# wangchou/whisper.coreml

Hardware: AMD Instinct MI355X
Metric: xRT (audio-s/s) large-v3 beam=5 @1/2/4/8 GPU; p50 per-token decode ms (higher is better)
Workload: dtype fp16; 1 GPU; large-v3 beam=5 transcribe() of one 600 s file, 30 s clip grid, condition_on_previous_text=False, temperature=0; model=large-v3, global_batch=20, seq_len=448

## Files before the change

### include/whisper_hip.h

```cpp
#ifndef WHISPER_HIP_H
#define WHISPER_HIP_H
#include <stdint.h>

#ifdef __cplusplus
extern "C" {
#endif

typedef struct wh_ctx wh_ctx;

typedef struct wh_dims {
  int n_mels, n_audio_ctx, n_audio_state, n_audio_head, n_audio_layer;
  int n_vocab, n_text_ctx, n_text_state, n_text_head, n_text_layer;
} wh_dims;

enum { WH_F32 = 0, WH_F16 = 1 };

typedef struct wh_decode_opts {
  int group;
  int beam;
  float patience;
  float temperature;
  int sample_len;
  int suppress_blank;
  int timestamps;
// ... 46 lines not shown
int wh_mel_max_batch(wh_ctx* ctx, float* gmax, int n_files);
int wh_mel_read(wh_ctx* ctx, float* out, int64_t frame0, int64_t n_frames);
int wh_mel_write(wh_ctx* ctx, const float* mel, int64_t n_frames);

int wh_encode(wh_ctx* ctx, int n_win, const int64_t* seek_frames, const int* seg_frames);
int wh_read_audio_features(wh_ctx* ctx, int slot, float* out);
int wh_read_cross_kv(wh_ctx* ctx, int slot, int layer, float* k_out, float* v_out);

int wh_decode_begin(wh_ctx* ctx, int n_win, const wh_decode_opts* opts, const int* init_tokens, const int* n_init,
                    int max_init, const int* sot_index);
int wh_decode_begin_slots(wh_ctx* ctx, int n_win, const int* slots, const wh_decode_opts* opts,
                          const int* init_tokens, const int* n_init, int max_init, const int* sot_index);
int wh_decode_steps(wh_ctx* ctx, int max_steps, int* n_done);
int wh_decode_read(wh_ctx* ctx, int slot, int* tokens, float* sum_logprobs, int* len, int* fin_n, int* fin_tokens,
                   int* fin_len, float* fin_score, float* no_speech_prob);
int wh_decode_maxc(wh_ctx* ctx);

int wh_prefill(wh_ctx* ctx, int n_win, int group, const int* tokens, const int* n_tokens, int max_tokens,
               const int* sot_index, float* logits);
int wh_step(wh_ctx* ctx, const int* tokens, const int* text_offsets, float* logits);
int wh_reorder_kv(wh_ctx* ctx, const int* source_rows);

int wh_prefill_logits(wh_ctx* ctx, int slot, const int* tokens, int n_tokens, float* logits, const int* align_heads,
                      int n_align, float* align_qk);

int wh_align(wh_ctx* ctx, int slot, const int* tokens, int n_tokens, int n_sot, int num_frames, const int* align_heads,
             int n_align, int medfilt_width, float* token_probs, int* path, int* path_len);
int wh_align_batch(wh_ctx* ctx, int n_win, const int* slots, const int* tokens, const int* n_tokens, int n_sot,
                   const int* num_frames, const int* align_heads, int n_align, int medfilt_width, float* token_probs,
                   int* paths, int* path_lens);
// ... 43 lines not shown
```

### whisper.coreml_amd/csrc/wh_kernels.h

```cpp
#pragma once
#include "wh_common.h"

namespace wh {

constexpr int TKP = 1536;

template <typename T>
void launch_layernorm(const float* x, T* y, const float* g, const float* b, int rows, int n, float eps,
                      const int* rows_in, hipStream_t st);
template <typename T>
void launch_resid_ln(float* x, const float* part, int nsplit, int64_t part_stride, const float* bias, T* y,
                     const float* g, const float* b, int rows, int n, float eps, hipStream_t st, int slab_half = 0);
template <typename T>
void launch_attn_enc(const T* qkv, int ld, int ns, int H, int Tlen, int nwin, int64_t wsi, const T* vt, int tkp, T* out,
                     int64_t wso, hipStream_t st);
template <typename T>
void launch_self_attn(const T* q, int ldq, const T* kc, const T* vc, const int* rw, const int* rs, const int* rp,
                      const int* anc, int anc_beams, int nbeam, int H, int ctx, T* out, int ldo, int rows,
                      hipStream_t st);
template <typename T>
int launch_self_attn_qkv(const float* part, int nsplit, int64_t part_stride, const float* bqkv, int ns, T* kc, T* vc,
                          const int* rw, const int* rs, const int* rp, const int* anc, int anc_beams, int nbeam, int H,
                          int ctx, T* out, int ldo, int rows, hipStream_t st, int slab_half = 0);
template <typename T>
// ... 7 lines not shown
  const float* bias = nullptr;
  int max_rows = 0;
  float* split_rec = nullptr;
  int* split_cnt = nullptr;
  int max_pairs = 0;
  const void* qx = nullptr;
  const void* qwf = nullptr;
};
inline bool xattn_fused_q(int n, int rows_per_window, int elem_size) {
  return elem_size == 2 && n == 1280 && rows_per_window >= 1 && rows_per_window <= 8;
}
void launch_wq_frag(const void* w, void* f, int n, hipStream_t st);
constexpr int XREC = 16 * 64 + 32;
constexpr int XS_NSP = 24;
constexpr int XS_QP = 4;
int xattn_seg_grid(int npair, int nsp, int smax);
inline bool cross_attn_q_slabs(int z) { return z == 4 || z == 8 || z == 10; }
template <typename T>
void launch_cross_attn(const T* q, int ldq, const T* ck, const T* cv, int Tk, int H, int nsplit, int nwin,
                       const int* win_row0, const int* win_nrows, const int* win_slot, int64_t win_stride, float* po,
                       float* pm, float* pl, T* out, int ldo, int rows, float* qk_out, const int* qk_map, int qk_rows,
                       hipStream_t st, XQPart xq = XQPart());
template <typename T>
void launch_embed(const T* E, const T* P, int n, const int* row_tok, int* row_pos, const int* hist,
                  const int* cur_len, int G, int hctx, int pmax, float* x, int rows, hipStream_t st);
template <typename T>
void launch_mel_windows(const float* mel, int64_t ld_mel, int n_mels, const int64_t* seeks, const int* segs, T* melT,
                        int64_t win_stride, int rows_alloc, int nwin, hipStream_t st);
template <typename T>
void launch_zero_rows(T* buf, int64_t ws, int n, int ra, int rb, int nwin, hipStream_t st);

// ... 68 lines not shown
```

### whisper.coreml_amd/csrc/wh_kernels.hip

```cpp
#include "wh_kernels.h"

#include <cstdio>
#include <type_traits>
#include <cstdlib>

namespace wh {

template <typename T>
__global__ __launch_bounds__(256) void k_layernorm(const float* __restrict__ x, T* __restrict__ y, const float* __restrict__ gamma,
                                                   const float* __restrict__ beta, int rows, int n, float eps,
                                                   const int* __restrict__ rows_in) {
  const int row = blockIdx.x * 4 + (threadIdx.x >> 6);
  const int lane = threadIdx.x & 63;
  if (row >= rows) return;
  const int src = rows_in ? rows_in[row] : row;
  const float* xr = x + (int64_t)src * n;
  constexpr int MAXV = 8;
  float4_t v[MAXV];
  const int nv = n >> 2;
#pragma unroll
  for (int i = 0; i < MAXV; ++i) {
    const int c = lane + 64 * i;
    if (c < nv) v[i] = load4f(xr + 4 * c);
  }
// ... 538 lines not shown
    store4(op, o[0] * inv, o[1] * inv, o[2] * inv, o[3] * inv);
    store4(op + 4, o[4] * inv, o[5] * inv, o[6] * inv, o[7] * inv);
  }
  CT_END(CT_SELF_ATTN);
}

template <typename T>
void launch_self_attn(const T* q, int ldq, const T* kc, const T* vc, const int* rw, const int* rs, const int* rp,
                      const int* anc, int anc_beams, int nbeam, int H, int ctx, T* out, int ldo, int rows,
                      hipStream_t st) {
  if (rows <= 0) return;
  k_self_attn<T><<<dim3(rows, H), 64, 0, st>>>(q, ldq, kc, vc, rw, rs, rp, anc, anc_beams, nbeam, H, ctx, out, ldo,
                                               self_attn_kco_min()), wh_launched("k_self_attn");
}

template <typename T, typename S = float>
__global__ __launch_bounds__(64) __attribute__((amdgpu_waves_per_eu(1, 2))) void k_self_attn_qkv(const S* __restrict__ part, int nsplit, int64_t part_stride,
                                                      const float* __restrict__ bqkv, int ns, T* __restrict__ kc,
                                                      T* __restrict__ vc, const int* __restrict__ row_win,
                                                      const int* __restrict__ row_slot, const int* __restrict__ row_pos,
                                                      const int* __restrict__ anc, int anc_beams, int nbeam, int H,
                                                      int ctx, T* __restrict__ out, int ldo, int kco_min = 0) {
  __shared__ float sc[512];
  __shared__ int slot_of[512];
  __shared__ float qs[64], vs[64];
  const int lane = threadIdx.x, G = anc_beams;
  CT_MARK(CT_SELF_ATTN, 0);
  const int L = xcd_remap(blockIdx.x, gridDim.x), sl = L % G, wh = L / G, h = wh % H, w = wh / H, row = w * G + sl;
  const int* an = anc + ((int64_t)w * anc_beams + sl) * ctx;
  const int64_t head_stride = (int64_t)ctx * 64;
  const int64_t wbase = (int64_t)w * nbeam;
  auto kv_off = [&](int slot, int p) -> int64_t { return ((wbase + slot) * H + h) * head_stride + (int64_t)p * 64; };
  constexpr int TB = (int)sizeof(T), ROWB = 64 * TB;
  const int slotB = H * ctx * ROWB, baseB = ((int)wbase * H + h) * ctx * ROWB;
  const auto rk = wt_rsrc(kc), rv = wt_rsrc(vc);
  const int pos = row_pos[row];
  int sv[8];
#pragma unroll
  for (int i = 0; i < 8; ++i) sv[i] = an[min(lane + 64 * i, ctx - 1)];
  float qd, kd, vd;
  {
    constexpr bool H16 = sizeof(S) == 2;
    const S* pr = part + (int64_t)row * 3 * ns + h * 64 + lane;
    qd = bqkv[h * 64 + lane];
    kd = bqkv[ns + h * 64 + lane];
    vd = bqkv[2 * ns + h * 64 + lane];
    S a0[16], a1[16], a2[16];
#pragma unroll
    for (int z = 0; z < 16; ++z)
      if (H16 || z < nsplit) {
        const int64_t zo = (int64_t)(H16 ? min(z, nsplit - 1) : z) * part_stride;
        a0[z] = pr[zo];
        a1[z] = pr[zo + ns];
        a2[z] = pr[zo + 2 * ns];
      }
    if constexpr (H16) {
      asm volatile("" ::"s"(pos));
#pragma unroll
      for (int z = 0; z < 16; ++z) asm volatile("" ::"v"(a0[z]), "v"(a1[z]), "v"(a2[z]));
    }
    auto f32 = [](S r) -> float { return (float)r; };
#pragma unroll
    for (int z = 0; z < 16; ++z)
      if (z < nsplit) {
        qd += f32(a0[z]);
        kd += f32(a1[z]);
        vd += f32(a2[z]);
      }
  }
  for (int i = 0; i < 8; ++i)
    if (lane + 64 * i < pos) slot_of[lane + 64 * i] = sv[i] * slotB;
  const int plast = max(pos - 1, 0);
  const T qT = from_f32<T>(qd), kT = from_f32<T>(kd), vT = from_f32<T>(vd);
  kc[kv_off(sl, pos) + lane] = kT;
  vc[kv_off(sl, pos) + lane] = vT;
  qs[lane] = to_f32(qT);
  vs[lane] = to_f32(vT);
  const float s_cur = wave_sum(to_f32(qT) * to_f32(kT));
// ... 170 lines not shown
int self_attn_kco_min() {
  static const int v = [] {
    const char* e = tune_env("WHISPER_HIP_SA_KCO_MIN");
    return e ? atoi(e) : 64;
  }();
  return v;
}
template <typename T>
int launch_self_attn_qkv(const float* part, int nsplit, int64_t part_stride, const float* bqkv, int ns, T* kc, T* vc,
                          const int* rw, const int* rs, const int* rp, const int* anc, int anc_beams, int nbeam, int H,
                          int ctx, T* out, int ldo, int rows, hipStream_t st, int slab_half) {
  if (rows <= 0) return 0;
  if (anc_beams < 1 || rows % anc_beams || nsplit > 16) return -1;
  if (slab_half) {
    if constexpr (sizeof(T) == 2) {
      k_self_attn_qkv<T, half_t><<<rows * H, 64, 0, st>>>(reinterpret_cast<const half_t*>(part), nsplit, part_stride,
                                                         bqkv, ns, kc, vc, rw, rs, rp, anc, anc_beams, nbeam, H, ctx,
                                                         out, ldo, self_attn_kco_min()), wh_launched("k_self_attn_qkv");
      return 0;
    }
    return -1;
  }
  k_self_attn_qkv<T><<<rows * H, 64, 0, st>>>(part, nsplit, part_stride, bqkv, ns, kc, vc, rw, rs, rp, anc, anc_beams,
                                             nbeam, H, ctx, out, ldo, self_attn_kco_min()), wh_launched("k_self_attn_qkv");
  return 0;
}

template <typename T, int ACT, typename S = float>
__global__ __launch_bounds__(256) void k_reduce_store(const S* __restrict__ part, int nsplit, int64_t part_stride,
                                                      const float* __restrict__ bias, T* __restrict__ out, int ldo, int M,
                                                      int N) {
  const int i = (int)(blockIdx.x * 256 + threadIdx.x) * 4;
  CT_MARK(CT_REDUCE, 0);
// ... 340 lines not shown
  }
  XS_MARK(8);
  wh_lds_barrier();
  if (kh == 0) {
    const float* bl = reinterpret_cast<const float*>(xst + BIAS_OFF);
#pragma unroll
    for (int j = 0; j < XS_QF; ++j)
      if (j < np) {
        float4_t v = red2[(j * 4 + c) * 64 + lane] + red2[((XS_QF + j) * 4 + c) * 64 + lane];
        v += *reinterpret_cast<const float4_t*>(bl + j * 64 + c * 16 + 4 * g);
        store4(&qs[j][r][c * 16 + 4 * g], v[0], v[1], v[2], v[3]);
      }
  }
}

template <typename T, int QZ, int RR, typename S = float, bool FULL = false, int QK = 0>
__global__ __launch_bounds__(512, 1) void k_xattn_seg(const T* __restrict__ q, int ldq, const T* ck, const T* cvt, int Tk,
                                                     int H, int npair, int nsp, const int* __restrict__ win_row0,
                                                     const int* __restrict__ win_nrows,
                                                     const int* __restrict__ win_slot, int64_t win_stride, XQPart xq,
                                                     T* __restrict__ out, int ldo) {
  constexpr int NW = 8, SMAX = XsShape<RR>::SMAX, PPASS = 512 / (RR * 16);
  constexpr bool QP = QZ > 0;
  constexpr bool QF = QK > 0;
  __shared__ float seg_m[SMAX][RR], seg_l[SMAX][RR];
  __shared__ __attribute__((aligned(16))) float seg_o[SMAX][RR][68];
  __shared__ __attribute__((aligned(16))) T qs[XS_QP][16][72];
  __shared__ int s_ticket[2];
  __shared__ int s_wnr[XS_QP], s_wr0[XS_QP];
  const int tid = threadIdx.x, lane = tid & 63, wave = tid >> 6;
  const int r = lane & 15, g = lane >> 4;
// ... 186 lines not shown
  XS_MARK(3);

  typedef unsigned u32x4 __attribute__((ext_vector_type(4)));
  const auto rs = __builtin_amdgcn_make_buffer_rsrc(xq.split_rec, 0, 0x7fffffff, 0x00020000);
  const int part = tid / (RR * 16), t = tid - part * (RR * 16), qq = t >> 4, dc = (t & 15) * 4;
  auto emit = [&](int pj, const float4_t& o) {
    int wj, hj;
    pair_wh(pj, wj, hj);
    store4(out + (int64_t)(s_wr0[pj - pa] + qq) * ldo + hj * 64 + dc, o[0], o[1], o[2], o[3]);
  };
#pragma unroll
  for (int pass = 0; pass < (XS_QP + PPASS - 1) / PPASS; ++pass) {
    const int pj = pa + pass * PPASS + part;
    if (pj <= plast && qq < s_wnr[pj - pa]) {
      const int l0 = pj * nsp - s0, l1 = l0 + nsp;
      if (l0 >= 0 && l1 <= cnt) {
        emit(pj, xs_merge(nsp, [&](int k, float& m, float& l, float4_t& o) {
               m = seg_m[l0 + k][qq];
               l = seg_l[l0 + k][qq];
               o = *reinterpret_cast<const float4_t*>(&seg_o[l0 + k][qq][dc]);
             }));
      } else {
        for (int s = max(l0, 0); s < min(l1, cnt); ++s) {
          const int rb = (pj * nsp + (s - l0)) * XREC * 4;
          const float4_t o = *reinterpret_cast<const float4_t*>(&seg_o[s][qq][dc]);
          __builtin_amdgcn_raw_buffer_store_b128(__builtin_bit_cast(u32x4, o), rs, rb + (qq * 64 + dc) * 4, 0, 16);
          if (dc == 0) {
            __builtin_amdgcn_raw_buffer_store_b32(__builtin_bit_cast(unsigned, seg_m[s][qq]), rs, rb + (1024 + qq) * 4, 0, 16);
            __builtin_amdgcn_raw_buffer_store_b32(__builtin_bit_cast(unsigned, seg_l[s][qq]), rs, rb + (1040 + qq) * 4, 0, 16);
          }
        }
      }
    }
  }
  asm volatile("s_waitcnt vmcnt(0)" ::: "memory");
  __syncthreads();
  XS_MARK(4);
  const bool cut_a = pa * nsp < s0 || pa * nsp + nsp > s1;
  const bool cut_b = plast != pa && plast * nsp + nsp > s1;
  if (tid == 0) {
    const int ca = min(s1, pa * nsp + nsp) - s0, cb = s1 - plast * nsp;
    s_ticket[0] = cut_a && __hip_atomic_fetch_add(xq.split_cnt + pa, ca, __ATOMIC_RELAXED, __HIP_MEMORY_SCOPE_AGENT) + ca == nsp;
    s_ticket[1] = cut_b && __hip_atomic_fetch_add(xq.split_cnt + plast, cb, __ATOMIC_RELAXED, __HIP_MEMORY_SCOPE_AGENT) + cb == nsp;
  }
  __syncthreads();
  XS_MARK(5);
  CT_MARK(CT_XATTN, 3);
  if (part > 1 || !s_ticket[part]) return;
  __builtin_amdgcn_fence(__ATOMIC_ACQUIRE, "wavefront");
// ... 6 lines not shown
         l = __builtin_bit_cast(float, __builtin_amdgcn_raw_buffer_load_b32(rs, rb + (1040 + qq) * 4, 0, 16));
         o = __builtin_bit_cast(float4_t, __builtin_amdgcn_raw_buffer_load_b128(rs, rb + (qq * 64 + dc) * 4, 0, 16));
       }));
  XS_MARK(6);
}

#if WH_TUNING
}
WH_CT_READER(kernels)
extern "C" int wh_tune_xs_trace(unsigned long long* out) {
  return hipMemcpyFromSymbol(out, HIP_SYMBOL(wh::g_xs_trace), sizeof(wh::g_xs_trace)) == hipSuccess ? 0 : -1;
}
namespace wh {
#endif

int xattn_seg_grid(int npair, int nsp, int smax) {
  const int nseg = npair * nsp;
  int k = (nseg + 256 * 8 - 1) / (256 * 8), forced = 0;
  if (const char* e = tune_env("WHISPER_HIP_XS_K")) {
    const int v = atoi(e);
    if (v >= 1) k = v, forced = 1;
    if (v < 0) {
      const int nwg = std::min(-v, nseg);
      return (nseg + nwg - 1) / nwg > smax ? (nseg + smax - 1) / smax : nwg;
    }
  }
  if (!forced && npair >= 192) {
    const int ppw = (npair + 255) / 256, nwg = (npair + ppw - 1) / ppw;
    if (nwg >= 192 && ppw * nsp <= smax) return nwg;
  }
  if (k > smax / 8) k = smax / 8;
  int nwg = k == 1 ? (nseg < 200 ? nseg : 200) : (nseg + 8 * k - 1) / (8 * k);
  if ((nseg + nwg - 1) / nwg > smax) nwg = (nseg + smax - 1) / smax;
  return nwg;
}

__global__ __launch_bounds__(256) void k_wq_frag(const half_t* __restrict__ w, half_t* __restrict__ f, int n) {
  const int QK = n / 64, total = n * n / 8;
  for (int i = blockIdx.x * 256 + threadIdx.x; i < total; i += gridDim.x * 256) {
    const int l = i % 64, t0 = i / 64, s = t0 % QK, t1 = t0 / QK, kh = t1 % 2, t2 = t1 / 2, c = t2 % 4, h = t2 / 4;
    const int row = h * 64 + c * 16 + (l & 15), col = kh * (n / 2) + 32 * s + 8 * (l >> 4);
    *reinterpret_cast<float4_t*>(f + (int64_t)i * 8) = *reinterpret_cast<const float4_t*>(w + (int64_t)row * n + col);
  }
}
void launch_wq_frag(const void* w, void* f, int n, hipStream_t st) {
  k_wq_frag<<<256, 256, 0, st>>>(reinterpret_cast<const half_t*>(w), reinterpret_cast<half_t*>(f), n), wh_launched("k_wq_frag");
}

template <typename T>
void launch_cross_attn(const T* q, int ldq, const T* ck, const T* cv, int Tk, int H, int nsplit, int nwin,
                       const int* win_row0, const int* win_nrows, const int* win_slot, int64_t win_stride, float* po,
                       float* pm, float* pl, T* out, int ldo, int rows, float* qk_out, const int* qk_map, int qk_rows,
                       hipStream_t st, XQPart xq) {
  if (rows <= 0) return;
  const int nsp = (Tk + 63) / 64;
  if (xq.max_rows >= 1 && xq.max_rows <= 16 && !qk_map && xq.split_rec && xq.split_cnt && nsp <= XS_NSP &&
      nwin * H <= xq.max_pairs) {
    const int npair = nwin * H;
    const int nwg_xs = xattn_seg_grid(npair, nsp, xq.max_rows <= 8 ? XsShape<8>::SMAX : XsShape<16>::SMAX);
    const bool full = (npair * nsp) / nwg_xs >= 8;
    if (xq.part_half && sizeof(T) != 2) {
      wh_set_launch_error("launch_cross_attn: fp16 query slabs in an fp32 context");
      return;
    }
    if (xq.qx) {
      if constexpr (sizeof(T) == 2) {
        if (!xq.qwf || !xq.bias || !xattn_fused_q(H * 64, xq.max_rows, (int)sizeof(T)) || nsp != XS_NSP) {
          wh_set_launch_error("launch_cross_attn: fused query projection outside its shapes");
          return;
        }
#define XQF(FULL_)                                                                                            \
  k_xattn_seg<T, 0, 8, float, FULL_, 20><<<nwg_xs, 512, 0, st>>>(q, ldq, ck, cv, Tk, H, npair, nsp, win_row0, \
                                                                 win_nrows, win_slot, win_stride, xq, out, ldo), \
      wh_launched("k_xattn_seg<qproj>")
        if (full) XQF(true);
        else XQF(false);
#undef XQF
      } else {
        wh_set_launch_error("launch_cross_attn: fused query projection in an fp32 context");
      }
      return;
    }
#define XSF(QZ_, RR_, S_)                                                                                         \
  if (full)                                                                                                     \
    k_xattn_seg<T, QZ_, RR_, S_, true><<<nwg_xs, 512, 0, st>>>(q, ldq, ck, cv, Tk, H, npair, nsp, win_row0,       \
                                                               win_nrows, win_slot, win_stride, xq, out, ldo), wh_launched("k_xattn_seg");   \
  else                                                                                                          \
    k_xattn_seg<T, QZ_, RR_, S_, false><<<nwg_xs, 512, 0, st>>>(q, ldq, ck, cv, Tk, H, npair, nsp, win_row0,      \
                                                                win_nrows, win_slot, win_stride, xq, out, ldo), wh_launched("k_xattn_seg")
#define XS(QZ_, RR_)                          \
  if constexpr (sizeof(T) == 2 && QZ_ > 0) {  \
    if (xq.part_half) {                       \
      XSF(QZ_, RR_, half_t);                  \
      return;                                 \
    }                                         \
  }                                           \
  XSF(QZ_, RR_, float)
#define XSR(QZ_)                        \
  if (xq.max_rows <= 8) {               \
// ... 259 lines not shown
```

### whisper.coreml_amd/csrc/wh_runtime.hip

```cpp
#include <hip/hip_runtime.h>

#include <algorithm>
#include <chrono>
#include <cmath>
#include <cstdio>
#include <cstring>
#include <set>
#include <string>
#include <vector>

#include "whisper_hip.h"
#include "wh_align.h"
#include "wh_audio.h"
#include "wh_gemm.h"
#include "wh_host.h"
#include "wh_kernels.h"

using namespace wh;

static thread_local std::string g_release_error;

namespace {

constexpr int CTX = 448;
// ... 44 lines not shown
  virtual ~wh_ctx() {}
  virtual int load(const std::string& name, const float* data, const int64_t* shape, int ndim) = 0;
  virtual int finalize() = 0;
  virtual int encode(int n_win, const int64_t* seeks, const int* segs) = 0;
  virtual int read_xa(int slot, float* out) = 0;
  virtual int read_ckv(int slot, int layer, float* k, float* v) = 0;
  virtual int decode_begin(int n_win, const wh_decode_opts* o, const int* init, const int* n_init, int max_init,
                           const int* sot_index, const int* slots) = 0;
  virtual int decode_steps(int max_steps, int* n_done) = 0;
  virtual int step_prefill(int n_win, int G, const int* init, const int* n_init, int max_init, const int* sot_index,
                           float* lg) = 0;
  virtual int step_tokens(const int* tok, const int* offsets, float* lg) = 0;
  virtual int reorder_kv(const int* src) = 0;
  virtual int decode_read(int slot, int* tokens, float* slp, int* len, int* fin_n, int* fin_tok, int* fin_len,
                          float* fin_score, float* nsp) = 0;
  virtual int prefill_logits(int slot, const int* tokens, int n, float* logits, const int* ah, int na, float* aqk) = 0;
  virtual int align(int slot, const int* tokens, int n, int n_sot, int num_frames, const int* ah, int na, int medfilt,
                    float* probs, int* path, int* plen) = 0;
  virtual int align_batch(int n_win, const int* slots, const int* tokens, const int* n_tokens, int n_sot,
                          const int* num_frames, const int* ah, int na, int medfilt, float* probs, int* paths,
                          int* plens) = 0;
  virtual int dtw(const float* x, int N, int M, int* path, int* plen) = 0;
  virtual int time_stage(int what, int iters, double* ms) = 0;
  virtual int share_weights_from(wh_ctx* src) = 0;
  int sharers = 0;
  wh_ctx* shares_from = nullptr;
  std::vector<float> token_ms;
  double stats[WH_N_STATS] = {0};
  AudioFront audio;
  int n_mels = 0;
// ... 51 lines not shown
    xq.max_rows = rows_per_window;
    xq.split_rec = xs_rec;
    xq.split_cnt = xs_cnt;
    xq.max_pairs = Wcap * nh;
    return xq;
  }
  int* qk_map;
  unsigned* suppress;
  DecState S;
  DecOpts O;
  int cur_nwin = 0, cur_G = 1;
  hipGraph_t graph = nullptr;
  hipGraphExec_t gexec = nullptr;
  std::vector<char> graph_key;
  int* h_done = nullptr;
  hipEvent_t poll_ev[2] = {nullptr, nullptr};

  Timer tm;
  std::vector<hipEvent_t> proj_ev;
  int proj_ev_n = 0;

  int share_weights_from(wh_ctx* src_) override {
    auto* src = dynamic_cast<Ctx<T>*>(src_);
    if (!src || src->ns != ns || src->Ld != Ld || src->La != La || src->V != V || !src->finalized)
      return fail(-2, "share_weights: a finalized context of the same dims and dtype is needed");
    conv1_w = src->conv1_w; conv2_w = src->conv2_w; E = src->E; Pdec = src->Pdec; ckv_w = src->ckv_w;
    conv1_b = src->conv1_b; conv2_b = src->conv2_b; pos_enc = src->pos_enc; lnp_g = src->lnp_g; lnp_b = src->lnp_b;
    ln_g = src->ln_g; ln_b = src->ln_b; ckv_b = src->ckv_b;
    enc = src->enc;
    dec = src->dec;
// ... 3 lines not shown
    ++src->sharers;
    return 0;
  }

  Releases rel;
  ~Ctx() override {
    if (st) rel(hipStreamSynchronize(st), "hipStreamSynchronize");
    if (gexec) rel(hipGraphExecDestroy(gexec), "hipGraphExecDestroy");
    if (graph) rel(hipGraphDestroy(graph), "hipGraphDestroy");
    if (st) rel(hipStreamDestroy(st), "hipStreamDestroy");
    if (wbase) rel(hipFree(wbase), "hipFree(weights)");
    if (abase) rel(hipFree(abase), "hipFree(activations)");
    audio.release(rel);
    scratch.release(rel, "hipFree(scratch)");
    if (h_done) rel(hipHostFree(h_done), "hipHostFree(done flags)");
    for (auto& e : poll_ev)
      if (e) rel(hipEventDestroy(e), "hipEventDestroy(poll)");
    tm.release(rel);
    (void)hipGetLastError();
    if (!rel.first.empty()) g_release_error = rel.first;
  }

  int init(int device_, const wh_dims& dims, int Wcap_, int Gcap_) {
    device = device_;
    d = dims;
    ns = d.n_text_state;
    nh = d.n_text_head;
    La = d.n_audio_layer;
    Ld = d.n_text_layer;
    V = d.n_vocab;
    n_mels = d.n_mels;
    if (d.n_audio_state != ns || d.n_audio_head != nh) return fail(-2, "audio/text state or head mismatch unsupported");
    if (ns != nh * 64) return fail(-2, "head dim must be 64 (decoder.py:62-64)");
    if (d.n_audio_ctx != 1500 || d.n_text_ctx != CTX) return fail(-2, "n_audio_ctx must be 1500, n_text_ctx 448");
    if (ns % 128 || ns > 2048) return fail(-2, "n_state must be a multiple of 128 and <= 2048");
    if (V > 57344) return fail(-2, "n_vocab too large");
    Wcap = Wcap_;
    Gcap = Gcap_;
    if (Wcap < 1 || Gcap < 1 || Gcap > 8) return fail(-2, "bad max_windows / max_group");
    const int kb = 128 / (int)sizeof(T);
    K1p = ((3 * n_mels + kb - 1) / kb) * kb;
    HIPCHK(hipSetDevice(device));
    HIPCHK(hipStreamCreateWithFlags(&st, hipStreamNonBlocking));
    TRY(tm.create());
    HIPCHK(hipHostMalloc((void**)&h_done, sizeof(int) * 2 * Wcap));
    for (auto& e : poll_ev) HIPCHK(hipEventCreateWithFlags(&e, hipEventDisableTiming));
    const size_t n = ns;
    size_t wb = 0;
    auto add = [&](size_t elems, size_t esz) { wb += ((elems * esz + 255) & ~size_t(255)) + 256; };
    add(n * K1p, sizeof(T)); add(n, 4); add(n * 3 * n, sizeof(T)); add(n, 4); add(1500 * n, 4);
    for (int l = 0; l < La; ++l) {
      add(n, 4); add(n, 4); add(3 * n * n, sizeof(T)); add(3 * n, 4); add(n * n, sizeof(T)); add(n, 4);
      add(n, 4); add(n, 4); add(4 * n * n, sizeof(T)); add(4 * n, 4); add(4 * n * n, sizeof(T)); add(n, 4);
    }
    add(n, 4); add(n, 4);
    add((size_t)V * n, sizeof(T)); add(CTX * n, sizeof(T));
    for (int l = 0; l < Ld; ++l) {
      add(n, 4); add(n, 4); add(3 * n * n, sizeof(T)); add(3 * n, 4); add(n * n, sizeof(T)); add(n, 4);
      add(n, 4); add(n, 4); add(n * n, sizeof(T)); add(n, 4); add(n * n, sizeof(T)); add(n, 4);
      add(n, 4); add(n, 4); add(4 * n * n, sizeof(T)); add(4 * n, 4); add(4 * n * n, sizeof(T)); add(n, 4);
// ... 521 lines not shown
        {att_d, n, e.wox, n},     {xn_d, n, e.w1, 4 * n}, {hm_d, 4 * n, e.w2, n}};
    for (auto& p : ps) {
      if (p.W == e.wqx && xq_proj_active(cur_G)) continue;
      int ks = 0;
      TRY(partial(p.X, p.K, p.W, R, p.N, p.K, &ks));
    }
    return 0;
  }

  bool p1_active(int R, int n_win) const { return n_win == 1 && p1_enabled() && proj1_supported(R, ns); }
  std::string step_kernels(int n_win, int group) const override {
    const bool p1 = p1_active(n_win * group, n_win), h = sizeof(T) == 2;
    return std::string("proj=") + (p1 ? "k_proj1" : "k_proj") + ",xattn=k_xattn_seg" +
           (!p1 && xq_proj_active(group) ? "<qproj>" : "") + ",self_attn=" +
           (p1 ? (h ? "k_self_attn<kco>" : "k_self_attn") : h ? "k_self_attn_qkv<pipe+kco>" : "k_self_attn_qkv") +
           ",tail=vocab+k_logit_part";
  }

  int dec_layers_p1(int R, const int* rw, const int* rs, const int* rp, int ancG, int nwin, const int* wr0,
                    const int* wnr, const int* wsl, const int* A) {
    const int n = ns;
    float* xc = x_d;
    float* xo = x2_d;
    const float* pend = nullptr;
    auto ln_in = [&](GemmArgs& g, const float* lg, const float* lb) {
      g.xf32 = xc; g.ln_g = lg; g.ln_b = lb; g.ln_eps = 1e-5f;
      if (pend) { g.res_slab = p1_slab; g.res_bias = pend; g.x_out = xo; }
    };
    auto ln_done = [&]() {
      if (pend) { std::swap(xc, xo); pend = nullptr; }
    };
// ... 360 lines not shown

  int decode_read(int slot, int* tokens, float* slp, int* len, int* fin_n, int* fin_tok, int* fin_len,
                  float* fin_score, float* nspo) override {
    if (slot < 0 || slot >= cur_nwin) return fail(-14, "slot");
    const int G = cur_G;
    HIPCHK(hipStreamSynchronize(st));
    if (tokens) HIPCHK(hipMemcpy(tokens, S.hist + (size_t)slot * G * HCTX, (size_t)G * HCTX * 4, hipMemcpyDeviceToHost));
    if (slp) HIPCHK(hipMemcpy(slp, S.sum_lp + slot * G, G * 4, hipMemcpyDeviceToHost));
    if (len) HIPCHK(hipMemcpy(len, S.len + slot, 4, hipMemcpyDeviceToHost));
    if (fin_n) HIPCHK(hipMemcpy(fin_n, S.fin_n + slot, 4, hipMemcpyDeviceToHost));
    const int mc = S.maxc;
    if (fin_tok) HIPCHK(hipMemcpy(fin_tok, S.fin_tok + (size_t)slot * mc * HCTX, (size_t)mc * HCTX * 4, hipMemcpyDeviceToHost));
    if (fin_len) HIPCHK(hipMemcpy(fin_len, S.fin_len + slot * mc, mc * 4, hipMemcpyDeviceToHost));
    if (fin_score) HIPCHK(hipMemcpy(fin_score, S.fin_score + slot * mc, mc * 4, hipMemcpyDeviceToHost));
    if (nspo) HIPCHK(hipMemcpy(nspo, nsp + slot, 4, hipMemcpyDeviceToHost));
    return 0;
  }

  int check_slot_idle(int slot) {
    if (cur_nwin < 1 || step_api) return 0;
    for (int w = 0; w < cur_nwin; ++w)
      if (win_slots[w] == slot) {
        int d = 0;
        HIPCHK(hipMemcpyAsync(&d, S.done + w, 4, hipMemcpyDeviceToHost, st));
        HIPCHK(hipStreamSynchronize(st));
        if (!d)
          return fail(-15, "slot " + std::to_string(slot) + " is still decoding (window " + std::to_string(w) +
                               " of the current batch): a first pass would overwrite its self-KV rows");
      }
    return 0;
// ... 437 lines not shown
int wh_mel_write(wh_ctx* ctx, const float* mel, int64_t nf) { CTXCALL(ctx->audio.mel_write(mel, nf, ctx->n_mels)); }
int wh_encode(wh_ctx* ctx, int n_win, const int64_t* seeks, const int* segs) { CTXCALL(ctx->encode(n_win, seeks, segs)); }
int wh_read_audio_features(wh_ctx* ctx, int slot, float* out) { CTXCALL(ctx->read_xa(slot, out)); }
int wh_read_cross_kv(wh_ctx* ctx, int slot, int layer, float* k, float* v) { CTXCALL(ctx->read_ckv(slot, layer, k, v)); }
int wh_decode_begin(wh_ctx* ctx, int n_win, const wh_decode_opts* o, const int* init, const int* n_init, int max_init,
                    const int* sot_index) {
  if (!o || !init || !n_init || !sot_index) return fail(-1, "null argument");
  CTXCALL(ctx->decode_begin(n_win, o, init, n_init, max_init, sot_index, nullptr));
}
int wh_decode_begin_slots(wh_ctx* ctx, int n_win, const int* slots, const wh_decode_opts* o, const int* init,
                          const int* n_init, int max_init, const int* sot_index) {
  if (!slots || !o || !init || !n_init || !sot_index) return fail(-1, "null argument");
  CTXCALL(ctx->decode_begin(n_win, o, init, n_init, max_init, sot_index, slots));
}
int wh_decode_steps(wh_ctx* ctx, int max_steps, int* n_done) { CTXCALL(ctx->decode_steps(max_steps, n_done)); }
int wh_decode_read(wh_ctx* ctx, int slot, int* tokens, float* slp, int* len, int* fin_n, int* fin_tok, int* fin_len,
                   float* fin_score, float* nsp) {
  CTXCALL(ctx->decode_read(slot, tokens, slp, len, fin_n, fin_tok, fin_len, fin_score, nsp));
}
int wh_decode_maxc(wh_ctx* ctx) { return ctx ? ctx->maxc_stride : -1; }
int wh_prefill(wh_ctx* ctx, int n_win, int group, const int* tokens, const int* n_tokens, int max_tokens,
               const int* sot_index, float* logits) {
  if (!tokens || !n_tokens || !sot_index) return fail(-1, "null argument");
  CTXCALL(ctx->step_prefill(n_win, group, tokens, n_tokens, max_tokens, sot_index, logits));
}
int wh_step(wh_ctx* ctx, const int* tokens, const int* text_offsets, float* logits) {
  if (!tokens) return fail(-1, "null argument");
  CTXCALL(ctx->step_tokens(tokens, text_offsets, logits));
}
int wh_reorder_kv(wh_ctx* ctx, const int* source_rows) {
// ... 49 lines not shown
```

### whisper.coreml_amd/whisper/backend_hip.py

```python

import ctypes
import os
from ctypes import POINTER, c_char_p, c_double, c_float, c_int, c_int64, c_uint64, c_void_p
from typing import NamedTuple, Optional, Sequence

import numpy as np

_PKG_DIR = os.path.dirname(os.path.abspath(__file__))
_DEFAULT_LIB = os.path.join(os.path.dirname(_PKG_DIR), "lib", "libwhisper_hip.so")

WH_F32 = 0
WH_F16 = 1
WH_PCM_S16, WH_PCM_S32, WH_PCM_F32 = 0, 1, 2


class HipBackendError(RuntimeError):
    pass


class WhDims(ctypes.Structure):
    _fields_ = [(k, c_int) for k in ("n_mels", "n_audio_ctx", "n_audio_state", "n_audio_head", "n_audio_layer",
                                     "n_vocab", "n_text_ctx", "n_text_state", "n_text_head", "n_text_layer")]


# ... 45 lines not shown
    "wh_mel_max": (c_int, [c_void_p, POINTER(c_float)]),
    "wh_mel_normalize": (c_int, [c_void_p, c_float]),
    "wh_log_mel_batch": (c_int, [c_void_p, c_void_p, c_int, c_void_p, c_int64, c_int, c_void_p]),
    "wh_mel_max_batch": (c_int, [c_void_p, c_void_p, c_int]),
    "wh_mel_read": (c_int, [c_void_p, c_void_p, c_int64, c_int64]),
    "wh_mel_write": (c_int, [c_void_p, c_void_p, c_int64]),
    "wh_encode": (c_int, [c_void_p, c_int, c_void_p, c_void_p]),
    "wh_read_audio_features": (c_int, [c_void_p, c_int, c_void_p]),
    "wh_read_cross_kv": (c_int, [c_void_p, c_int, c_int, c_void_p, c_void_p]),
    "wh_decode_begin": (c_int, [c_void_p, c_int, POINTER(WhDecodeOpts), c_void_p, c_void_p, c_int, c_void_p]),
    "wh_decode_begin_slots": (c_int, [c_void_p, c_int, c_void_p, POINTER(WhDecodeOpts), c_void_p, c_void_p, c_int,
                                      c_void_p]),
    "wh_decode_steps": (c_int, [c_void_p, c_int, POINTER(c_int)]),
    "wh_decode_read": (c_int, [c_void_p, c_int, c_void_p, c_void_p, c_void_p, c_void_p, c_void_p, c_void_p,
                               c_void_p, c_void_p]),
    "wh_decode_maxc": (c_int, [c_void_p]),
    "wh_prefill": (c_int, [c_void_p, c_int, c_int, c_void_p, c_void_p, c_int, c_void_p, c_void_p]),
    "wh_step": (c_int, [c_void_p, c_void_p, c_void_p, c_void_p]),
    "wh_reorder_kv": (c_int, [c_void_p, c_void_p]),
    "wh_prefill_logits": (c_int, [c_void_p, c_int, c_void_p, c_int, c_void_p, c_void_p, c_int, c_void_p]),
    "wh_align": (c_int, [c_void_p, c_int, c_void_p, c_int, c_int, c_int, c_void_p, c_int, c_int, c_void_p, c_void_p,
                         POINTER(c_int)]),
    "wh_align_batch": (c_int, [c_void_p, c_int, c_void_p, c_void_p, c_void_p, c_int, c_void_p, c_void_p, c_int,
                               c_int, c_void_p, c_void_p, c_void_p]),
    "wh_dtw": (c_int, [c_void_p, c_void_p, c_int, c_int, c_void_p, POINTER(c_int)]),
    "wh_stats": (c_int, [c_void_p, POINTER(c_double), c_int]),
    "wh_sync": (c_int, [c_void_p]),
    "wh_time_stage": (c_int, [c_void_p, c_int, c_int, POINTER(c_double)]),
    "wh_step_kernels": (c_int, [c_void_p, c_int, c_int, ctypes.c_char_p, c_int]),
    "wh_token_ms": (c_int, [c_void_p, c_void_p, c_int, POINTER(c_int), c_int]),
# ... 368 lines not shown
        maxc = max(1, self.lib.wh_decode_maxc(self.h))
        toks = np.zeros((group, hctx), dtype=np.int32)
        slp = np.zeros(group, dtype=np.float32)
        ln = np.zeros(1, dtype=np.int32)
        fn = np.zeros(1, dtype=np.int32)
        ftok = np.zeros((maxc, hctx), dtype=np.int32)
        flen = np.zeros(maxc, dtype=np.int32)
        fsc = np.zeros(maxc, dtype=np.float32)
        nsp = np.zeros(1, dtype=np.float32)
        self._check(self.lib.wh_decode_read(self.h, slot, _ptr(toks), _ptr(slp), _ptr(ln), _ptr(fn), _ptr(ftok),
                                            _ptr(flen), _ptr(fsc), _ptr(nsp)), "wh_decode_read")
        n = int(fn[0])
        return dict(tokens=toks, sum_logprobs=slp, length=int(ln[0]), fin_tokens=ftok[:n], fin_len=flen[:n],
                    fin_score=fsc[:n], no_speech_prob=float(nsp[0]))

    def prefill(self, init_tokens: Sequence[Sequence[int]], group: int, sot_index: Sequence[int],
                logits: bool = True):
        n = len(init_tokens)
        mx = max(len(t) for t in init_tokens)
        arr = np.zeros((n, mx), dtype=np.int32)
        for i, t in enumerate(init_tokens):
            arr[i, :len(t)] = t
        nin = np.asarray([len(t) for t in init_tokens], dtype=np.int32)
        si = np.asarray(sot_index, dtype=np.int32)
        out = np.empty((n, 2, self.dims["n_vocab"]), dtype=np.float32) if logits else None
        self._check(self.lib.wh_prefill(self.h, n, int(group), _ptr(arr), _ptr(nin), mx, _ptr(si),
                                        _ptr(out) if out is not None else None), "wh_prefill")
        return out

    def step(self, tokens: Sequence[int], text_offsets: Optional[Sequence[int]] = None, logits: bool = True):
# ... 88 lines not shown
```

### whisper.coreml_amd/whisper/decoding.py

```python

import itertools
import zlib
from dataclasses import dataclass, field, replace
from typing import TYPE_CHECKING, Dict, Iterable, List, Optional, Sequence, Tuple, Union

import numpy as np

from .audio import CHUNK_LENGTH, N_FRAMES
from .backend_hip import WhDecodeOpts
from .tokenizer import Tokenizer, get_tokenizer

if TYPE_CHECKING:
    from .model import Whisper

_seed_counter = itertools.count(1)


def next_seed() -> int:
    return next(_seed_counter) * 0x9E3779B97F4A7C15 % (1 << 64)


def compression_ratio(text: str) -> float:
    b = text.encode("utf-8")
    return len(b) / len(zlib.compress(b)) if b else 0.0
# ... 150 lines not shown
                audio_features: bool = False, slots: Optional[Sequence[int]] = None,
                languages: Optional[Sequence[Optional[str]]] = None, seed: Optional[int] = None
                ) -> List[DecodingResult]:
    if languages is None:
        tasks = [DecodingTask(model, replace(options, prompt=p)) for p in prompts]
    else:
        if len(languages) != len(prompts):
            raise ValueError("run_windows: one language per window")
        tasks = [DecodingTask(model, replace(options, prompt=p, language=lg)) for p, lg in zip(prompts, languages)]
    t0 = tasks[0]
    opts = t0.wh_opts(seed)
    ctx = model.ctx
    ctx.decode_begin(opts, [t.initial_tokens for t in tasks], [t.sot_index for t in tasks], slots=slots)
    ctx.decode_steps(t0.sample_len)
    out = []
    for i, t in enumerate(tasks):
        lang = t.tokenizer.language or "en"
        raw = ctx.decode_read(i, t.n_group)
        toks, _, avg = t.finalize(raw)
        text = t.tokenizer.decode(toks).strip()
        out.append(DecodingResult(
            audio_features=ctx.audio_features(slots[i] if slots is not None else i) if audio_features else None,
            language=lang, tokens=toks,
            text=text, avg_logprob=avg, no_speech_prob=raw["no_speech_prob"], temperature=options.temperature,
            compression_ratio=compression_ratio(text)))
    return out


def decode(model: "Whisper", mel, options: DecodingOptions = DecodingOptions(), **kwargs
           ) -> Union[DecodingResult, List[DecodingResult]]:
    mel = np.asarray(mel.detach().cpu().numpy() if hasattr(mel, "detach") else mel, dtype=np.float32)
    single = mel.ndim == 2
    if single:
# ... 50 lines not shown
```

Before: 761.3 audio-s/s.

## Batch decode read-back, specialize QKV slab count, add whole-segment xattn path

```diff
diff --git a/include/whisper_hip.h b/include/whisper_hip.h
--- a/include/whisper_hip.h
+++ b/include/whisper_hip.h
@@ -84,6 +84,8 @@
 int wh_decode_steps(wh_ctx* ctx, int max_steps, int* n_done);
 int wh_decode_read(wh_ctx* ctx, int slot, int* tokens, float* sum_logprobs, int* len, int* fin_n, int* fin_tokens,
                    int* fin_len, float* fin_score, float* no_speech_prob);
+int wh_decode_read_all(wh_ctx* ctx, int n_win, int* tokens, float* sum_logprobs, int* len, int* fin_n,
+                       int* fin_tokens, int* fin_len, float* fin_score, float* no_speech_prob);
 int wh_decode_maxc(wh_ctx* ctx);
 
 int wh_prefill(wh_ctx* ctx, int n_win, int group, const int* tokens, const int* n_tokens, int max_tokens,
diff --git a/whisper.coreml_amd/csrc/wh_kernels.h b/whisper.coreml_amd/csrc/wh_kernels.h
--- a/whisper.coreml_amd/csrc/wh_kernels.h
+++ b/whisper.coreml_amd/csrc/wh_kernels.h
@@ -45,7 +45,7 @@
 constexpr int XREC = 16 * 64 + 32;
 constexpr int XS_NSP = 24;
 constexpr int XS_QP = 4;
-int xattn_seg_grid(int npair, int nsp, int smax);
+int xattn_seg_grid(int npair, int nsp, int smax, bool* whole = nullptr);
 inline bool cross_attn_q_slabs(int z) { return z == 4 || z == 8 || z == 10; }
 template <typename T>
 void launch_cross_attn(const T* q, int ldq, const T* ck, const T* cv, int Tk, int H, int nsplit, int nwin,
diff --git a/whisper.coreml_amd/csrc/wh_kernels.hip b/whisper.coreml_amd/csrc/wh_kernels.hip
--- a/whisper.coreml_amd/csrc/wh_kernels.hip
+++ b/whisper.coreml_amd/csrc/wh_kernels.hip
@@ -576,7 +576,7 @@
                                                self_attn_kco_min()), wh_launched("k_self_attn");
 }
 
-template <typename T, typename S = float>
+template <typename T, typename S = float, int NS = 16>
 __global__ __launch_bounds__(64) __attribute__((amdgpu_waves_per_eu(1, 2))) void k_self_attn_qkv(const S* __restrict__ part, int nsplit, int64_t part_stride,
                                                       const float* __restrict__ bqkv, int ns, T* __restrict__ kc,
                                                       T* __restrict__ vc, const int* __restrict__ row_win,
@@ -607,9 +607,9 @@
     qd = bqkv[h * 64 + lane];
     kd = bqkv[ns + h * 64 + lane];
     vd = bqkv[2 * ns + h * 64 + lane];
-    S a0[16], a1[16], a2[16];
-#pragma unroll
-    for (int z = 0; z < 16; ++z)
+    S a0[NS], a1[NS], a2[NS];
+#pragma unroll
+    for (int z = 0; z < NS; ++z)
       if (H16 || z < nsplit) {
         const int64_t zo = (int64_t)(H16 ? min(z, nsplit - 1) : z) * part_stride;
         a0[z] = pr[zo];
@@ -619,11 +619,11 @@
     if constexpr (H16) {
       asm volatile("" ::"s"(pos));
 #pragma unroll
-      for (int z = 0; z < 16; ++z) asm volatile("" ::"v"(a0[z]), "v"(a1[z]), "v"(a2[z]));
+      for (int z = 0; z < NS; ++z) asm volatile("" ::"v"(a0[z]), "v"(a1[z]), "v"(a2[z]));
     }
     auto f32 = [](S r) -> float { return (float)r; };
 #pragma unroll
-    for (int z = 0; z < 16; ++z)
+    for (int z = 0; z < NS; ++z)
       if (z < nsplit) {
         qd += f32(a0[z]);
         kd += f32(a1[z]);
@@ -824,9 +824,19 @@
   if (anc_beams < 1 || rows % anc_beams || nsplit > 16) return -1;
   if (slab_half) {
     if constexpr (sizeof(T) == 2) {
-      k_self_attn_qkv<T, half_t><<<rows * H, 64, 0, st>>>(reinterpret_cast<const half_t*>(part), nsplit, part_stride,
-                                                         bqkv, ns, kc, vc, rw, rs, rp, anc, anc_beams, nbeam, H, ctx,
-                                                         out, ldo, self_attn_kco_min()), wh_launched("k_self_attn_qkv");
+      const half_t* ph = reinterpret_cast<const half_t*>(part);
+#define SAQ(NS_)                                                                                                      \
+  k_self_attn_qkv<T, half_t, NS_><<<rows * H, 64, 0, st>>>(ph, nsplit, part_stride, bqkv, ns, kc, vc, rw, rs, rp, anc, \
+                                                           anc_beams, nbeam, H, ctx, out, ldo, self_attn_kco_min()),   \
+      wh_launched("k_self_attn_qkv")
+      static const bool by_count = [] {
+        const char* e = tune_env("WHISPER_HIP_SA_NS");
+        return !(e && e[0] == '0');
+      }();
+      if (by_count && nsplit <= 4) SAQ(4);
+      else if (by_count && nsplit <= 8) SAQ(8);
+      else SAQ(16);
+#undef SAQ
       return 0;
     }
     return -1;
@@ -1197,7 +1207,7 @@
   }
 }
 
-template <typename T, int QZ, int RR, typename S = float, bool FULL = false, int QK = 0>
+template <typename T, int QZ, int RR, typename S = float, bool FULL = false, int QK = 0, bool WHOLE = false>
 __global__ __launch_bounds__(512, 1) void k_xattn_seg(const T* __restrict__ q, int ldq, const T* ck, const T* cvt, int Tk,
                                                      int H, int npair, int nsp, const int* __restrict__ win_row0,
                                                      const int* __restrict__ win_nrows,
@@ -1414,7 +1424,7 @@
     const int pj = pa + pass * PPASS + part;
     if (pj <= plast && qq < s_wnr[pj - pa]) {
       const int l0 = pj * nsp - s0, l1 = l0 + nsp;
-      if (l0 >= 0 && l1 <= cnt) {
+      if (WHOLE || (l0 >= 0 && l1 <= cnt)) {
         emit(pj, xs_merge(nsp, [&](int k, float& m, float& l, float4_t& o) {
                m = seg_m[l0 + k][qq];
                l = seg_l[l0 + k][qq];
@@ -1433,6 +1443,10 @@
       }
     }
   }
+  if constexpr (WHOLE) {
+    CT_MARK(CT_XATTN, 3);
+    return;
+  }
   asm volatile("s_waitcnt vmcnt(0)" ::: "memory");
   __syncthreads();
   XS_MARK(4);
@@ -1469,7 +1483,8 @@
 namespace wh {
 #endif
 
-int xattn_seg_grid(int npair, int nsp, int smax) {
+int xattn_seg_grid(int npair, int nsp, int smax, bool* whole) {
+  if (whole) *whole = false;
   const int nseg = npair * nsp;
   int k = (nseg + 256 * 8 - 1) / (256 * 8), forced = 0;
   if (const char* e = tune_env("WHISPER_HIP_XS_K")) {
@@ -1482,7 +1497,10 @@
   }
   if (!forced && npair >= 192) {
     const int ppw = (npair + 255) / 256, nwg = (npair + ppw - 1) / ppw;
-    if (nwg >= 192 && ppw * nsp <= smax) return nwg;
+    if (nwg >= 192 && ppw * nsp <= smax) {
+      if (whole) *whole = npair % ppw == 0;
+      return nwg;
+    }
   }
   if (k > smax / 8) k = smax / 8;
   int nwg = k == 1 ? (nseg < 200 ? nseg : 200) : (nseg + 8 * k - 1) / (8 * k);
@@ -1512,8 +1530,14 @@
   if (xq.max_rows >= 1 && xq.max_rows <= 16 && !qk_map && xq.split_rec && xq.split_cnt && nsp <= XS_NSP &&
       nwin * H <= xq.max_pairs) {
     const int npair = nwin * H;
-    const int nwg_xs = xattn_seg_grid(npair, nsp, xq.max_rows <= 8 ? XsShape<8>::SMAX : XsShape<16>::SMAX);
+    bool whole = false;
+    const int nwg_xs = xattn_seg_grid(npair, nsp, xq.max_rows <= 8 ? XsShape<8>::SMAX : XsShape<16>::SMAX, &whole);
     const bool full = (npair * nsp) / nwg_xs >= 8;
+    static const bool whole_on = [] {
+      const char* e = tune_env("WHISPER_HIP_XS_WHOLE");
+      return !(e && e[0] == '0');
+    }();
+    whole = whole && whole_on && full;
     if (xq.part_half && sizeof(T) != 2) {
       wh_set_launch_error("launch_cross_attn: fp16 query slabs in an fp32 context");
       return;
@@ -1524,12 +1548,14 @@
           wh_set_launch_error("launch_cross_attn: fused query projection outside its shapes");
           return;
         }
-#define XQF(FULL_)                                                                                            \
-  k_xattn_seg<T, 0, 8, float, FULL_, 20><<<nwg_xs, 512, 0, st>>>(q, ldq, ck, cv, Tk, H, npair, nsp, win_row0, \
-                                                                 win_nrows, win_slot, win_stride, xq, out, ldo), \
+#define XQF(FULL_, WHOLE_)                                                                                            \
+  k_xattn_seg<T, 0, 8, float, FULL_, 20, WHOLE_><<<nwg_xs, 512, 0, st>>>(q, ldq, ck, cv, Tk, H, npair, nsp, win_row0, \
+                                                                         win_nrows, win_slot, win_stride, xq, out,    \
+                                                                         ldo),                                        \
       wh_launched("k_xattn_seg<qproj>")
-        if (full) XQF(true);
-        else XQF(false);
+        if (whole) XQF(true, true);
+        else if (full) XQF(true, false);
+        else XQF(false, false);
 #undef XQF
       } else {
         wh_set_launch_error("launch_cross_attn: fused query projection in an fp32 context");
@@ -1537,7 +1563,10 @@
       return;
     }
 #define XSF(QZ_, RR_, S_)                                                                                         \
-  if (full)                                                                                                     \
+  if (whole)                                                                                                    \
+    k_xattn_seg<T, QZ_, RR_, S_, true, 0, true><<<nwg_xs, 512, 0, st>>>(q, ldq, ck, cv, Tk, H, npair, nsp, win_row0, \
+                                                                        win_nrows, win_slot, win_stride, xq, out, ldo), wh_launched("k_xattn_seg"); \
+  else if (full)                                                                                                \
     k_xattn_seg<T, QZ_, RR_, S_, true><<<nwg_xs, 512, 0, st>>>(q, ldq, ck, cv, Tk, H, npair, nsp, win_row0,       \
                                                                win_nrows, win_slot, win_stride, xq, out, ldo), wh_launched("k_xattn_seg");   \
   else                                                                                                          \
diff --git a/whisper.coreml_amd/csrc/wh_runtime.hip b/whisper.coreml_amd/csrc/wh_runtime.hip
--- a/whisper.coreml_amd/csrc/wh_runtime.hip
+++ b/whisper.coreml_amd/csrc/wh_runtime.hip
@@ -82,6 +82,8 @@
   virtual int reorder_kv(const int* src) = 0;
   virtual int decode_read(int slot, int* tokens, float* slp, int* len, int* fin_n, int* fin_tok, int* fin_len,
                           float* fin_score, float* nsp) = 0;
+  virtual int decode_read_all(int n_win, int* tokens, float* slp, int* len, int* fin_n, int* fin_tok, int* fin_len,
+                              float* fin_score, float* nsp) = 0;
   virtual int prefill_logits(int slot, const int* tokens, int n, float* logits, const int* ah, int na, float* aqk) = 0;
   virtual int align(int slot, const int* tokens, int n, int n_sot, int num_frames, const int* ah, int na, int medfilt,
                     float* probs, int* path, int* plen) = 0;
@@ -163,6 +165,7 @@
   hipGraphExec_t gexec = nullptr;
   std::vector<char> graph_key;
   int* h_done = nullptr;
+  char* h_read = nullptr;
   hipEvent_t poll_ev[2] = {nullptr, nullptr};
 
   Timer tm;
@@ -196,6 +199,7 @@
     audio.release(rel);
     scratch.release(rel, "hipFree(scratch)");
     if (h_done) rel(hipHostFree(h_done), "hipHostFree(done flags)");
+    if (h_read) rel(hipHostFree(h_read), "hipHostFree(read-back)");
     for (auto& e : poll_ev)
       if (e) rel(hipEventDestroy(e), "hipEventDestroy(poll)");
     tm.release(rel);
@@ -226,6 +230,7 @@
     HIPCHK(hipStreamCreateWithFlags(&st, hipStreamNonBlocking));
     TRY(tm.create());
     HIPCHK(hipHostMalloc((void**)&h_done, sizeof(int) * 2 * Wcap));
+    HIPCHK(hipHostMalloc((void**)&h_read, read_all_bytes(Wcap, Gcap, 16)));
     for (auto& e : poll_ev) HIPCHK(hipEventCreateWithFlags(&e, hipEventDisableTiming));
     const size_t n = ns;
     size_t wb = 0;
@@ -777,7 +782,7 @@
     return std::string("proj=") + (p1 ? "k_proj1" : "k_proj") + ",xattn=k_xattn_seg" +
            (!p1 && xq_proj_active(group) ? "<qproj>" : "") + ",self_attn=" +
            (p1 ? (h ? "k_self_attn<kco>" : "k_self_attn") : h ? "k_self_attn_qkv<pipe+kco>" : "k_self_attn_qkv") +
-           ",tail=vocab+k_logit_part";
+           ",tail=vocab+k_logit_part,read=wh_decode_read_all,qkv_slabs=" + std::to_string(sa_probe_ks);
   }
 
   int dec_layers_p1(int R, const int* rw, const int* rs, const int* rp, int ancG, int nwin, const int* wr0,
@@ -1168,6 +1173,34 @@
     if (fin_len) HIPCHK(hipMemcpy(fin_len, S.fin_len + slot * mc, mc * 4, hipMemcpyDeviceToHost));
     if (fin_score) HIPCHK(hipMemcpy(fin_score, S.fin_score + slot * mc, mc * 4, hipMemcpyDeviceToHost));
     if (nspo) HIPCHK(hipMemcpy(nspo, nsp + slot, 4, hipMemcpyDeviceToHost));
+    return 0;
+  }
+
+  static size_t read_all_bytes(int nw, int G, int mc) {
+    return (size_t)nw * ((size_t)G * HCTX + G + 2 + (size_t)mc * HCTX + 2 * mc + 1) * 4;
+  }
+  int decode_read_all(int n_win, int* tokens, float* slp, int* len, int* fin_n, int* fin_tok, int* fin_len,
+                      float* fin_score, float* nspo) override {
+    if (cur_nwin < 1 || n_win != cur_nwin) return fail(-14, "n_win is not the current batch's window count");
+    const size_t W = n_win, G = cur_G, mc = S.maxc;
+    struct Part { void* dst; const void* src; size_t bytes; };
+    const Part parts[8] = {{tokens, S.hist, W * G * HCTX * 4}, {slp, S.sum_lp, W * G * 4},
+                           {len, S.len, W * 4},               {fin_n, S.fin_n, W * 4},
+                           {fin_tok, S.fin_tok, W * mc * HCTX * 4}, {fin_len, S.fin_len, W * mc * 4},
+                           {fin_score, S.fin_score, W * mc * 4},    {nspo, nsp, W * 4}};
+    size_t off = 0;
+    for (const Part& p : parts) {
+      if (!p.dst) continue;
+      HIPCHK(hipMemcpyAsync(h_read + off, p.src, p.bytes, hipMemcpyDeviceToHost, st));
+      off += p.bytes;
+    }
+    HIPCHK(hipStreamSynchronize(st));
+    off = 0;
+    for (const Part& p : parts) {
+      if (!p.dst) continue;
+      memcpy(p.dst, h_read + off, p.bytes);
+      off += p.bytes;
+    }
     return 0;
   }
 
@@ -1635,6 +1668,10 @@
   CTXCALL(ctx->decode_begin(n_win, o, init, n_init, max_init, sot_index, slots));
 }
 int wh_decode_steps(wh_ctx* ctx, int max_steps, int* n_done) { CTXCALL(ctx->decode_steps(max_steps, n_done)); }
+int wh_decode_read_all(wh_ctx* ctx, int n_win, int* tokens, float* slp, int* len, int* fin_n, int* fin_tok,
+                       int* fin_len, float* fin_score, float* nsp) {
+  CTXCALL(ctx->decode_read_all(n_win, tokens, slp, len, fin_n, fin_tok, fin_len, fin_score, nsp));
+}
 int wh_decode_read(wh_ctx* ctx, int slot, int* tokens, float* slp, int* len, int* fin_n, int* fin_tok, int* fin_len,
                    float* fin_score, float* nsp) {
   CTXCALL(ctx->decode_read(slot, tokens, slp, len, fin_n, fin_tok, fin_len, fin_score, nsp));
diff --git a/whisper.coreml_amd/whisper/backend_hip.py b/whisper.coreml_amd/whisper/backend_hip.py
--- a/whisper.coreml_amd/whisper/backend_hip.py
+++ b/whisper.coreml_amd/whisper/backend_hip.py
@@ -83,6 +83,8 @@
     "wh_decode_steps": (c_int, [c_void_p, c_int, POINTER(c_int)]),
     "wh_decode_read": (c_int, [c_void_p, c_int, c_void_p, c_void_p, c_void_p, c_void_p, c_void_p, c_void_p,
                                c_void_p, c_void_p]),
+    "wh_decode_read_all": (c_int, [c_void_p, c_int, c_void_p, c_void_p, c_void_p, c_void_p, c_void_p, c_void_p,
+                                   c_void_p, c_void_p]),
     "wh_decode_maxc": (c_int, [c_void_p]),
     "wh_prefill": (c_int, [c_void_p, c_int, c_int, c_void_p, c_void_p, c_int, c_void_p, c_void_p]),
     "wh_step": (c_int, [c_void_p, c_void_p, c_void_p, c_void_p]),
@@ -481,6 +483,26 @@
         return dict(tokens=toks, sum_logprobs=slp, length=int(ln[0]), fin_tokens=ftok[:n], fin_len=flen[:n],
                     fin_score=fsc[:n], no_speech_prob=float(nsp[0]))
 
+    def decode_read_all(self, n_win: int, group: int):
+        hctx = self.dims["n_text_ctx"] + 1
+        maxc = max(1, self.lib.wh_decode_maxc(self.h))
+        toks = np.zeros((n_win, group, hctx), dtype=np.int32)
+        slp = np.zeros((n_win, group), dtype=np.float32)
+        ln = np.zeros(n_win, dtype=np.int32)
+        fn = np.zeros(n_win, dtype=np.int32)
+        ftok = np.zeros((n_win, maxc, hctx), dtype=np.int32)
+        flen = np.zeros((n_win, maxc), dtype=np.int32)
+        fsc = np.zeros((n_win, maxc), dtype=np.float32)
+        nsp = np.zeros(n_win, dtype=np.float32)
+        self._check(self.lib.wh_decode_read_all(self.h, int(n_win), _ptr(toks), _ptr(slp), _ptr(ln), _ptr(fn),
+                                                _ptr(ftok), _ptr(flen), _ptr(fsc), _ptr(nsp)), "wh_decode_read_all")
+        out = []
+        for w in range(n_win):
+            n = int(fn[w])
+            out.append(dict(tokens=toks[w], sum_logprobs=slp[w], length=int(ln[w]), fin_tokens=ftok[w, :n],
+                            fin_len=flen[w, :n], fin_score=fsc[w, :n], no_speech_prob=float(nsp[w])))
+        return out
+
     def prefill(self, init_tokens: Sequence[Sequence[int]], group: int, sot_index: Sequence[int],
                 logits: bool = True):
         n = len(init_tokens)
diff --git a/whisper.coreml_amd/whisper/decoding.py b/whisper.coreml_amd/whisper/decoding.py
--- a/whisper.coreml_amd/whisper/decoding.py
+++ b/whisper.coreml_amd/whisper/decoding.py
@@ -188,9 +188,10 @@
     ctx.decode_begin(opts, [t.initial_tokens for t in tasks], [t.sot_index for t in tasks], slots=slots)
     ctx.decode_steps(t0.sample_len)
     out = []
+    raws = ctx.decode_read_all(len(tasks), t0.n_group)
     for i, t in enumerate(tasks):
         lang = t.tokenizer.language or "en"
-        raw = ctx.decode_read(i, t.n_group)
+        raw = raws[i]
         toks, _, avg = t.finalize(raw)
         text = t.tokenizer.decode(toks).strip()
         out.append(DecodingResult(
```

Result: no change. 767.0 audio-s/s (median of 6 runs) (+0.8%).
